# Jackxiini/Pytorch-distributed-learning

Measured on AMD Instinct MI355X. Metric: images/sec (whole node) MNIST ConvNet at 1/2/4/8 MI355X; DDP scaling efficiency, higher is better.
Workload: dtype bf16

## Files before the change

### csrc/kernels/convnet_bwd12.hip

```cpp
#include "convnet_device.h"
#include "convnet_host.h"

namespace ringdp {
namespace kern {

namespace {

__device__ __forceinline__ bf16x8 ones_column_frag(int lane) {
  const bf16 one = (bf16)((lane & 15) == 0 ? 1.f : 0.f);
  return bf16x8{one, one, one, one, one, one, one, one};
}

constexpr int C2_PW = 15, C2_PRS = 80, C2_ORS = 40, C2_DRS = 72;
__constant__ uint8_t c2d_tile_pos[176] = {0,1,2,3,8,9,10,11,12,19,20,13,4,5,6,7,14,15,16,17,22,23,24,25,32,39,34,27,18,33,26,21,28,29,30,31,36,37,38,45,52,53,48,41,46,47,40,35,42,43,44,59,50,51,58,65,66,67,62,55,60,61,54,49,56,57,72,73,64,71,78,79,80,81,76,69,74,75,68,63,70,85,86,87,84,91,92,93,94,95,90,83,88,89,82,77,98,99,100,101,104,105,106,107,108,109,110,111,102,103,96,97,112,113,114,115,118,119,120,121,122,137,130,125,116,123,124,117,126,127,128,129,132,133,134,135,150,151,144,139,136,143,138,131,140,141,142,149,146,147,148,163,164,165,158,153,156,157,152,145,154,155,162,168,160,161,255,255,255,255,255,167,255,255,166,159};
constexpr int C2D_P = C2_PW * C2_PW * C2_PRS * 2;
constexpr int C2D_O = 169 * C2_ORS * 2;
__device__ __forceinline__ int c2_drow(int r) { return (r >> 3) * 704 + (r & 7) * 80; }
constexpr int C2W_D = 16 * 704 * 2;
constexpr int C2W_X = 169 * C2_XRS * 2;
constexpr int C2B_LDS = (C2D_P + 2 * C2D_O) > (C2W_D + C2W_X) ? (C2D_P + 2 * C2D_O) : (C2W_D + C2W_X);
constexpr int C2_WSLAB = 288 * 64 + 64;

__device__ __forceinline__ void conv2_dgrad_role(char* smem, const bf16* __restrict__ dz2, const bf16* __restrict__ packed,
                                 bf16* __restrict__ da1, int B, int block, int nblocks) {
  bf16* P = reinterpret_cast<bf16*>(smem);
  bf16* O = reinterpret_cast<bf16*>(smem + C2D_P);
  const int tid = threadIdx.x, lane = tid & 63, wave = tid >> 6;
  const int nt = wave & 1, mg = wave >> 1;
  const int r16 = lane & 15, q8 = (lane >> 4) * 8;
  const bf16x8* pk = reinterpret_cast<const bf16x8*>(packed + P2D_OFF);
  bf16x8 bw[18];
#pragma unroll
  for (int ks = 0; ks < 18; ++ks) bw[ks] = pk[(nt * 18 + ks) * 64 + lane];
  int base[3];
  int opos[3][4];
#pragma unroll
  for (int k = 0; k < 3; ++k) {
    const int mt = min(mg + 4 * k, 10);
    const int mm = c2d_tile_pos[mt * 16 + r16] == 255 ? 0 : c2d_tile_pos[mt * 16 + r16];
    base[k] = (mm / 13) * C2_PW + mm % 13;
#pragma unroll
    for (int i = 0; i < 4; ++i) opos[k][i] = c2d_tile_pos[mt * 16 + (lane >> 4) * 4 + i];
  }
  for (int c = tid; c < C2D_P / 16; c += 512) reinterpret_cast<bf16x8*>(P)[c] = zero_bf16x8();
  auto copy_out = [&](int bb, const bf16* src) {
    bf16x8* dst = reinterpret_cast<bf16x8*>(da1 + (int64_t)bb * 169 * 32);
    for (int c = tid; c < 676; c += 512) dst[c] = *reinterpret_cast<const bf16x8*>(src + (c >> 2) * C2_ORS + (c & 3) * 8);
  };
  bf16x8 pz[2];
  auto load = [&](int bb) {
    const bf16x8* src = reinterpret_cast<const bf16x8*>(dz2 + (int64_t)bb * 121 * 64);
    pz[0] = src[tid];
    if (tid + 512 < 968) pz[1] = src[tid + 512];
  };
  auto mfma_phase = [&](auto nk_c, bf16* Oc) {
    constexpr int NK = decltype(nk_c)::value;
    f32x4 acc[NK];
#pragma unroll
    for (int k = 0; k < NK; ++k) acc[k] = zero_f32x4();
#pragma unroll
    for (int ks = 0; ks < 18; ++ks) {
      const int tapp = ks >> 1, c0 = (ks & 1) * 32;
      const int shift = (tapp / 3) * C2_PW + tapp % 3;
#pragma unroll
      for (int k = 0; k < NK; ++k)
        acc[k] = mfma16x16x32(*reinterpret_cast<const bf16x8*>(P + (base[k] + shift) * C2_PRS + c0 + q8), bw[ks],
                              acc[k]);
    }
#pragma unroll
    for (int k = 0; k < NK; ++k) {
#pragma unroll
      for (int i = 0; i < 4; ++i) {
        const int m = opos[k][i];
        if (m < 169) Oc[m * C2_ORS + nt * 16 + r16] = (bf16)acc[k][i];
      }
    }
  };
  int b = block, prev = -1, cur = 0;
  if (b < B) load(b);
  for (; b < B; b += nblocks) {
    __syncthreads();
    if (prev >= 0) copy_out(prev, O + (cur ^ 1) * 169 * C2_ORS);
#pragma unroll
    for (int k = 0; k < 2; ++k) {
      const int c = tid + 512 * k;
      if (c < 968) {
        const int pos = c >> 3, cc = (c & 7) * 8;
        *reinterpret_cast<bf16x8*>(P + ((pos / 11 + 2) * C2_PW + pos % 11 + 2) * C2_PRS + cc) = pz[k];
      }
    }
    const int nb = b + nblocks;
    if (nb < B) load(nb);
    __syncthreads();
// ... 350 lines not shown
      if (mg < 3) phase(I3{}, T{}, k);
      else phase(I2{}, T{}, k);
    }
  }
  __syncthreads();
  if (b != block) {
#pragma unroll
    for (int j = 0; j < 4; ++j) c1_step(j, k ^ 1);
  }
  __syncthreads();
  float* red = reinterpret_cast<float*>(smem);
#pragma unroll
  for (int m = 0; m < 2; ++m)
#pragma unroll
    for (int n = 0; n < 2; ++n)
      *reinterpret_cast<f32x4*>(red + ((wave * 4 + m * 2 + n) * 64 + lane) * 4) = acc1[m][n];
  __syncthreads();
  if (tid >= 256) return;
  const int tile = tid >> 6;
  f32x4 sum = *reinterpret_cast<const f32x4*>(red + (tile * 64 + lane) * 4);
#pragma unroll
  for (int w = 1; w < 8; ++w) sum += *reinterpret_cast<const f32x4*>(red + ((w * 4 + tile) * 64 + lane) * 4);
  float* slab = slabs1 + (int64_t)block * C1_WSLAB;
  const int tap = (tile & 1) * 16 + i16;
#pragma unroll
  for (int r = 0; r < 4; ++r) {
    const int co = (tile >> 1) * 16 + g * 4 + r;
    if (tap < 25) slab[co * 25 + tap] = sum[r];
    if (tap == 25) slab[800 + co] = sum[r];
  }
}

template <bool U8>
__global__ __launch_bounds__(512) void conv12_bwd_kernel(const void* __restrict__ xin,
                                                         const uint8_t* __restrict__ idx1,
                                                         const bf16* __restrict__ a1,
                                                         const bf16* __restrict__ dz2,
                                                         const bf16* __restrict__ packed, int B,
                                                         float mean, float inv_std, float in_scale,
                                                         float* __restrict__ slabs2, int nslices,
                                                         float* __restrict__ slabs1, int n_dgrad) {
  __shared__ __attribute__((aligned(16))) char smem[C12B_LDS];
  if ((int)blockIdx.x < n_dgrad)
    conv12_dgrad_role<U8>(smem, xin, idx1, dz2, packed, B, blockIdx.x, n_dgrad, mean, inv_std, in_scale, slabs1);
  else
    conv2_wgrad_role(smem, a1, dz2, slabs2, B, nslices, blockIdx.x - n_dgrad);
}

constexpr int C12V_DG = 2 * (C2D_P + C12_O) + 3 * (C12_XS + C1I_IMG);
constexpr int C12V_WG = 3 * (C2W_D + C2W_X);
constexpr int C12V_LDS = C12V_DG > C12V_WG ? C12V_DG : C12V_WG;
static_assert(C12V_LDS <= 160 * 1024 && C1I_IMG % 16 == 0, "conv12 backward (8-wave) LDS");

#ifndef RINGDP_C12_ABLATE
#define RINGDP_C12_ABLATE 0
#endif
constexpr int C12_ABLATE = RINGDP_C12_ABLATE;

#ifdef RINGDP_C12_STAMPS
constexpr int C12_ST_S0 = 100, C12_ST_BLK = 5, C12_ST_BYTES = 8 * 8 * 4 * 8;
#define C12_ST(s, k) CN_STAMP(C12V_LDS, C12_ST_S0, 4, s, k)
#else
constexpr int C12_ST_BYTES = 0;
#define C12_ST(s, k) do {} while (0)
#endif

template <bool U8>
__device__ __forceinline__ void conv12_dgrad8_role(char* smem, const void* __restrict__ xin,
                                                   const uint8_t* __restrict__ idx1, const bf16* __restrict__ dz2,
                                                   const bf16* __restrict__ packed, int B, int block, int nblocks,
                                                   float mean, float inv_std, float in_scale,
                                                   float* __restrict__ slabs1, int ablate) {
  auto Pb = [&](int k) { return reinterpret_cast<bf16*>(smem + k * C2D_P); };
  auto Ob = [&](int k) { return reinterpret_cast<bf16*>(smem + 2 * C2D_P + k * C12_O); };
  auto Xb = [&](int k) { return reinterpret_cast<bf16*>(smem + 2 * (C2D_P + C12_O) + k * C12_XS); };
  auto Cb = [&](int k) { return reinterpret_cast<uint8_t*>(smem + 2 * (C2D_P + C12_O) + 3 * C12_XS + k * C1I_IMG); };
  const int tid = threadIdx.x, lane = tid & 63;
  const int wave = __builtin_amdgcn_readfirstlane(tid >> 6);
  const int n = block < B ? (B - block + nblocks - 1) / nblocks : 0;
  for (int c = tid; c < (2 * (C2D_P + C12_O) + 3 * C12_XS) / 16; c += 512)
    reinterpret_cast<bf16x8*>(smem)[c] = zero_bf16x8();
  __syncthreads();
  if ((ablate & 8) && wave >= 4) __builtin_amdgcn_s_setprio(1);
  constexpr int C12_KM = 2, C12_KM3 = 4, C12_KH = 26 - 3 * C12_KM - C12_KM3;
  static_assert(C12_KH >= 4 && C12_KM >= 0 && C12_KM3 >= 0, "conv1 k-step partition");
  const int k0 = wave < 4 ? C12_KH + wave * C12_KM : wave - 4, kst = wave < 4 ? 1 : 4;
  const int kcnt = wave < 3 ? C12_KM : wave == 3 ? C12_KM3 : (C12_KH - (wave - 4) + 3) / 4;
  const int i16 = lane & 15, g = lane >> 4, q = i16 >> 2, p = i16 & 3;
  const int t1 = 16 + i16;
  const int xoff0 = (i16 % 5) * C1W_CS + (i16 / 5) * C1W_RS + 8 * g;
  const int xoff1 = t1 < 25 ? (t1 % 5) * C1W_CS + (t1 / 5) * C1W_RS + 8 * g : 0;
  const uint32_t b1fill = t1 == 25 ? 0x3f803f80u : 0u;
  f32x4 acc1[2][2];
#pragma unroll
  for (int m = 0; m < 2; ++m) acc1[m][0] = acc1[m][1] = zero_f32x4();
  const int o_lane = ((4 * g + q) * C2_ORS + 4 * p) * 2;
  const int c_lane = (i16 >> 1) * 16 + 4 * g, csh_lane = 4 * (i16 & 1);
  struct C1F {
    uint2 d[2];
    uint32_t cu[2];
    bf16x8 b0, b1;
  };
  auto c1_read = [&](int ks, int oimg, int ximg, int cimg, C1F& f) {
    const int py = ks >> 1;
    int oa = oimg + py * (13 * C2_ORS * 2) + o_lane, ca = cimg + py * 256 + c_lane;
    int x0 = ximg + ks * (C1W_RS * 2) + xoff0 * 2, x1 = ximg + ks * (C1W_RS * 2) + xoff1 * 2;
    asm("" : "+v"(oa), "+v"(ca), "+v"(x0), "+v"(x1));
#pragma unroll
    for (int m = 0; m < 2; ++m) {
      f.d[m] = __builtin_bit_cast(uint2, lds_read_tr16(reinterpret_cast<const bf16*>(smem + oa) + m * 16));
      f.cu[m] = *reinterpret_cast<const uint32_t*>(smem + ca + m * 128);
    }
    f.b0 = *reinterpret_cast<const bf16x8*>(smem + x0);
    f.b1 = *reinterpret_cast<const bf16x8*>(smem + x1);
  };
  auto c1_mma = [&](int ks, const C1F& f) {
    bf16x8 A[2];
    const int csh = csh_lane + 2 * (ks & 1);
#pragma unroll
    for (int m = 0; m < 2; ++m) {
      const uint2 d = f.d[m];
      const uint32_t cu = f.cu[m];
      uint32_t pr[4];
#pragma unroll
      for (int e = 0; e < 4; ++e) {
        const uint32_t dv = e & 1 ? (e < 2 ? d.x : d.y) >> 16 : (e < 2 ? d.x : d.y) & 0xffffu;
        const uint32_t sel = __builtin_amdgcn_ubfe(cu, 8 * e + csh, 2);
        pr[e] = dv * ((sel * 0x8001u) & 0x10001u);
      }
      A[m] = __builtin_bit_cast(bf16x8, make_uint4(pr[0], pr[1], pr[2], pr[3]));
    }
    bf16x8 B1 = f.b1;
    if (t1 >= 25) B1 = __builtin_bit_cast(bf16x8, make_uint4(b1fill, b1fill, b1fill, b1fill));
#pragma unroll
    for (int m = 0; m < 2; ++m) {
      acc1[m][0] = mfma16x16x32(A[m], f.b0, acc1[m][0]);
      acc1[m][1] = mfma16x16x32(A[m], B1, acc1[m][1]);
    }
  };
  auto c1_image = [&](int j) {
    const int oimg = 2 * C2D_P + (j & 1) * C12_O;
    const int ximg = 2 * (C2D_P + C12_O) + (j % 3) * C12_XS;
    const int cimg = 2 * (C2D_P + C12_O) + 3 * C12_XS + (j % 3) * C1I_IMG;
    for (int i = 0, ks = k0; i < kcnt; ++i, ks += kst) {
      C1F f;
      c1_read(ks, oimg, ximg, cimg, f);
      c1_mma(ks, f);
    }
  };
  if (wave < 4) {
    const int r16 = lane & 15, q8 = (lane >> 4) * 8, c4 = (lane >> 4) * 4;
    const bf16x8* pk = reinterpret_cast<const bf16x8*>(packed + P2D_OFF);
    bf16x8 bw[2][18];
#pragma unroll
    for (int nt = 0; nt < 2; ++nt)
#pragma unroll
      for (int ks = 0; ks < 18; ++ks) bw[nt][ks] = pk[(nt * 18 + ks) * 64 + lane];
    int base[3], opos[3];
#pragma unroll
    for (int k = 0; k < 3; ++k) {
      const int mt = min(wave + 4 * k, 10);
      const int mm = c2d_tile_pos[mt * 16 + r16];
      opos[k] = mm;
      base[k] = mm == 255 ? 0 : (mm / 13) * C2_PW + mm % 13;
    }
    auto phase = [&](auto nk_c, const bf16* P, bf16* O, int s) {
      constexpr int NK = decltype(nk_c)::value;
      f32x4 acc[NK][2];
#pragma unroll
      for (int k = 0; k < NK; ++k) acc[k][0] = acc[k][1] = zero_f32x4();
#pragma unroll
      for (int ks = 0; ks < 18; ++ks) {
        const int tapp = ks >> 1, c0 = (ks & 1) * 32;
        const int shift = (tapp / 3) * C2_PW + tapp % 3;
#pragma unroll
        for (int k = 0; k < NK; ++k) {
          const bf16x8 a = *reinterpret_cast<const bf16x8*>(P + (base[k] + shift) * C2_PRS + c0 + q8);
          acc[k][0] = mfma16x16x32(bw[0][ks], a, acc[k][0]);
          acc[k][1] = mfma16x16x32(bw[1][ks], a, acc[k][1]);
        }
      }
      C12_ST(s, 1);
#pragma unroll
      for (int k = 0; k < NK; ++k) {
        if (opos[k] < 169) {
#pragma unroll
          for (int nt = 0; nt < 2; ++nt)
            *reinterpret_cast<bf16x4*>(O + opos[k] * C2_ORS + nt * 16 + c4) =
                bf16x4{(bf16)acc[k][nt][0], (bf16)acc[k][nt][1], (bf16)acc[k][nt][2], (bf16)acc[k][nt][3]};
        }
      }
    };
    lds_barrier();
    for (int s = 0; s <= n; ++s) {
      C12_ST(s, 0);
      if (s < n && !(ablate & 2)) {
        if (wave < 3)
          phase(std::integral_constant<int, 3>{}, Pb(s & 1), Ob(s & 1), s);
        else
          phase(std::integral_constant<int, 2>{}, Pb(s & 1), Ob(s & 1), s);
      }
      C12_ST(s, 2);
      if (s >= 1 && !(ablate & 1)) c1_image(s - 1);
      C12_ST(s, 3);
      lds_barrier();
    }
  } else {
    const int vt = tid - 256;
    struct Regs {
      bf16x8 pz[4];
      uint4 pc;
      uint32_t xu;
      float4 xf;
    };
    Regs r0, r1;
    auto load = [&](Regs& r, int bb) {
      const bf16x8* src = reinterpret_cast<const bf16x8*>(dz2 + (int64_t)bb * 121 * 64);
#pragma unroll
      for (int j = 0; j < 4; ++j)
        if (vt + 256 * j < 968) r.pz[j] = src[vt + 256 * j];
      if (vt < C1I_IMG / 16) r.pc = reinterpret_cast<const uint4*>(idx1 + (int64_t)bb * C1I_IMG)[vt];
      c1_load<U8>(xin, bb, vt, r.xu, r.xf);
    };
    auto stage = [&](const Regs& r, int k2, int k3) {
      bf16* P = Pb(k2);
#pragma unroll
      for (int j = 0; j < 4; ++j) {
        const int c = vt + 256 * j;
        if (c < 968) {
          const int pos = c >> 3, cc = (c & 7) * 8;
// ... 163 lines not shown
      C12_ST(i, 1);
      if (!early && i + 2 < n) {
        stage(rs, (i + 2) % 3);
        if (i + 4 < n) load(rs, img(i + 4));
      }
      lds_barrier();
      C12_ST(i, 2);
    };
    for (int i = 0; i < n; i += 2) {
      image(i, r0);
      if (i + 1 < n) image(i + 1, r1);
    }
  };
  if (h == 0)
    body(std::integral_constant<int, 0>{});
  else
    body(std::integral_constant<int, 1>{});
  float* slab = slabs + (int64_t)slice * C2_WSLAB;
  const int nj = h == 0 ? 5 : 4;
#pragma unroll
  for (int m = 0; m < 2; ++m) {
    const int co = (2 * wm2 + m) * 16 + grp * 4;
#pragma unroll
    for (int j = 0; j < 5; ++j) {
      if (j < nj) {
        const int nn = ((2 * j + h) * 2 + half) * 16 + g16;
        *reinterpret_cast<f32x4*>(slab + (int64_t)nn * 64 + co) = acc[m][j];
      }
    }
    if (wn == 0 && g16 == 0) *reinterpret_cast<f32x4*>(slab + 288 * 64 + co) = accb[m];
  }
}

template <bool U8>
__global__ __launch_bounds__(512, 1) void conv12_bwd8_kernel(const void* __restrict__ xin,
                                                            const uint8_t* __restrict__ idx1,
                                                            const bf16* __restrict__ a1,
                                                            const bf16* __restrict__ dz2,
                                                            const bf16* __restrict__ packed, int B, float mean,
                                                            float inv_std, float in_scale,
                                                            float* __restrict__ slabs2, int nslices,
                                                            float* __restrict__ slabs1, int n_dgrad, int ablate) {
  __shared__ __attribute__((aligned(16))) char smem[C12V_LDS + C12_ST_BYTES];
  if ((int)blockIdx.x < n_dgrad)
    conv12_dgrad8_role<U8>(smem, xin, idx1, dz2, packed, B, blockIdx.x, n_dgrad, mean, inv_std, in_scale, slabs1,
                           ablate);
  else if (!(ablate & 4))
    conv2_wgrad8_role(smem, a1, dz2, slabs2, B, nslices, blockIdx.x - n_dgrad);
#ifdef RINGDP_C12_STAMPS
  __syncthreads();
  const bool dg = (int)blockIdx.x < n_dgrad;
  const int blk = dg ? blockIdx.x : blockIdx.x - n_dgrad, nb = dg ? n_dgrad : nslices;
  if (blk == C12_ST_BLK && threadIdx.x == 0 && (B - blk) / nb > C12_ST_S0 + 8) {
    const unsigned long long* st = reinterpret_cast<const unsigned long long*>(smem + C12V_LDS);
    const unsigned long long t0 = st[0];
    for (int w = 0; w < 8; ++w)
      for (int k = 0; k < 8; ++k) {
        const unsigned long long* r = st + (w * 8 + k) * 4;
        printf("C12ST %c w%d s%d %lld %lld %lld %lld\n", dg ? 'd' : 'w', w, k, (long long)(r[0] - t0),
               (long long)(r[1] - t0), (long long)(r[2] - t0), dg ? (long long)(r[3] - t0) : 0ll);
      }
  }
#endif
}

}

static void c2_split(int B, bool dgrad, int& nd, int& ws) {
  const int cus = num_cus();
  if (!dgrad) {
    nd = 0;
    ws = clampi(cdiv(B, 8), 1, cus);
    return;
  }
  static const double frac = env_real("RINGDP_C2_DGRAD_FRAC", 0.55, split_frac_ok);
  nd = clampi(B, 1, (int)(frac * cus));
  const int per = cdiv(B, nd);
  ws = clampi(cdiv(B, std::max(per, 2)), 1, std::max(1, cus - nd));
}

static void c12_split(int B, int& nd, int& ws) {
  const int cus = num_cus();
  if (use_8wave(B)) {
    static const double frac3 = env_real("RINGDP_C12_DGRAD_FRAC", 0.59, split_frac_ok);
    nd = clampi(((int)(frac3 * cus) + 4) / 8 * 8, 8, cus - 8);
    ws = clampi(cdiv(B, 8), 1, cus - nd);
    return;
  }
  static const double frac = env_real("RINGDP_C12_DGRAD_FRAC", 0.64, split_frac_ok);
  static const int wmin = env_int("RINGDP_C12_WMIN", 2, slab_images_ok);
  nd = clampi(B, 1, (int)(frac * cus));
  const int per = cdiv(B, nd);
  ws = clampi(cdiv(B, std::max(per, wmin)), 1, std::max(1, cus - nd));
}

static int conv1_wslices(int B) { return clampi(cdiv(B, 4), 1, 3 * num_cus()); }

int64_t cn_conv2_slab_floats(int B, bool dgrad) {
  int nd, ws;
  c2_split(B, dgrad, nd, ws);
  return (int64_t)ws * C2_WSLAB;
}
int64_t cn_conv12_slab_floats(int B) {
  int nd, ws;
  c12_split(B, nd, ws);
  return (int64_t)ws * C2_WSLAB + (int64_t)nd * C1_WSLAB;
}
int64_t cn_conv1_slab_floats(int B) { return (int64_t)conv1_wslices(B) * C1_WSLAB; }

void cn_conv2_bwd(const void* a1, const void* dz2, const void* packed, void* da1, int B, float* slabs,
                  float* dw2, float* db2, hipStream_t s) {
  int nd, ws;
  c2_split(B, da1 != nullptr, nd, ws);
  conv2_bwd_kernel<<<nd + ws, 512, 0, s>>>(static_cast<const bf16*>(a1), static_cast<const bf16*>(dz2),
                                           static_cast<const bf16*>(packed), static_cast<bf16*>(da1), B, slabs,
                                           ws, nd);
  launch_reduce({seg(slabs, C2_WSLAB, 0, 288 * 64, ws, dw2, 1, 32, 64), seg(slabs, C2_WSLAB, 288 * 64, 64, ws, db2)},
                s);
}

void cn_conv12_bwd(const void* x, bool u8, const uint8_t* idx1, const void* a1, const void* dz2,
                   const void* packed, int B, float mean, float inv_std, float in_scale, float* slabs, float* dw2,
                   float* db2, float* dw1, float* db1, hipStream_t s, const ReduceList* extra) {
  int nd, ws;
  c12_split(B, nd, ws);
  float *slabs2 = slabs, *slabs1 = slabs + (int64_t)ws * C2_WSLAB;
  const bf16 *a1b = static_cast<const bf16*>(a1), *dzb = static_cast<const bf16*>(dz2),
             *pk = static_cast<const bf16*>(packed);
  dispatch_bool(u8, [&](auto U8) {
    if (use_8wave(B))
      conv12_bwd8_kernel<decltype(U8)::value><<<nd + ws, 512, 0, s>>>(x, idx1, a1b, dzb, pk, B, mean, inv_std, in_scale,
                                                                      slabs2, ws, slabs1, nd, C12_ABLATE);
    else
      conv12_bwd_kernel<decltype(U8)::value><<<nd + ws, 512, 0, s>>>(x, idx1, a1b, dzb, pk, B, mean, inv_std, in_scale,
                                                                     slabs2, ws, slabs1, nd);
  });
  ReduceList r = extra ? *extra : ReduceList{};
  for (const ReduceSeg& g : {seg(slabs2, C2_WSLAB, 0, 288 * 64, ws, dw2, 1, 32, 64),
                             seg(slabs2, C2_WSLAB, 288 * 64, 64, ws, db2), seg(slabs1, C1_WSLAB, 0, 800, nd, dw1),
                             seg(slabs1, C1_WSLAB, 800, 32, nd, db1)})
    r.push_back(g);
  launch_reduce(r, s);
}

void cn_conv1_wgrad(const void* x, bool u8, const void* da1, const uint8_t* idx1, int B, float mean,
                    float inv_std, float in_scale, float* slabs, float* dw1, float* db1, hipStream_t s) {
  const int ws = conv1_wslices(B);
  dispatch_bool(u8, [&](auto U8) {
    conv1_wgrad_kernel<decltype(U8)::value><<<ws, 256, 0, s>>>(x, static_cast<const bf16*>(da1), idx1, B, mean, inv_std,
                                                               in_scale, slabs, ws);
  });
  launch_reduce({seg(slabs, C1_WSLAB, 0, 800, ws, dw1), seg(slabs, C1_WSLAB, 800, 32, ws, db1)}, s);
}

}
}
```

### csrc/kernels/convnet_bwd3.hip

```cpp
#include "convnet_device.h"
#include "convnet_host.h"

namespace ringdp::kern {
namespace {
__host__ __device__ inline int fc_imgs(int B) { return B <= 1024 ? 4 : (B >= 65536 ? 128 : (B >= 32768 ? 64 : 32)); }
constexpr int FC_SLAB = 10 * 2048 + 10 + 128 + 2;

template <bool kCE>
__device__ __forceinline__ void fc_bwd_body(const bf16* __restrict__ a3, const bf16* __restrict__ packed,
                                            const float* __restrict__ dl, bf16* __restrict__ da3m,
                                            float* __restrict__ slabs, int B, int imgs, const CeFuse& ce, int blk) {
  const int t = threadIdx.x;
  const int wd = t >> 4, co0 = (t & 15) * 8;
  float wr[8][10];
  {
    const bf16x8* src = reinterpret_cast<const bf16x8*>(packed + PFC_OFF + (wd * 128 + co0) * 10);
#pragma unroll
    for (int h = 0; h < 10; ++h) {
      const bf16x8 v = src[h];
#pragma unroll
      for (int e = 0; e < 8; ++e) wr[(8 * h + e) / 10][(8 * h + e) % 10] = (float)v[e];
    }
  }
  float acc[8][10];
// ... 361 lines not shown
                                                           const uint8_t* __restrict__ idx3,
                                                           const bf16* __restrict__ packed, bf16* __restrict__ dz2,
                                                           int B, float* __restrict__ slabs, int n_wgrad,
                                                           int n_dgrad, int b_dgrad, int n_fc,
                                                           float* __restrict__ fc_slabs, int fc_n_imgs) {
  __shared__ __attribute__((aligned(16))) char smem[C3B_LDS];
  int blk = blockIdx.x;
  if (blk < n_fc) {
    if (src.dl)
      fc_bwd_body<false>(src.a3, packed, src.dl, nullptr, fc_slabs, B, fc_n_imgs, src.ce, blk);
    else
      fc_bwd_body<true>(src.a3, packed, nullptr, nullptr, fc_slabs, B, fc_n_imgs, src.ce, blk);
    return;
  }
  blk -= n_fc;
  int b_first = blk, b_end = b_dgrad, b_step = n_dgrad;
  if (blk >= n_dgrad) {
    const int w = blk - n_dgrad;
    conv3_wgrad_role(smem, a2, src, idx3, slabs, B, n_wgrad, w >> 1, w & 1);
    if (dz2 == nullptr || b_dgrad >= B) return;
    __syncthreads();
    b_first = b_dgrad + w;
    b_end = B;
    b_step = 2 * n_wgrad;
  }
  conv3_dgrad_role(smem, src, idx3, idx2, packed, dz2, b_first, b_end, b_step);
}

constexpr int C3S_B = 2048 * 2 + 2048;
constexpr int C3V_DA = 100 * 64 * 4;
constexpr int C3V_FV = 8 * 64 * 16;
constexpr int C3V_F = C3V_FV + 8 * 64 * 4;
constexpr int C3V_XRS = 80;
constexpr int C3V_X = 100 * C3V_XRS * 2;
constexpr int C3V_DG = 2 * (C3D_P + C3V_DA + C3D_AM + C3S_B);
constexpr int C3V_WG = 3 * C3V_X + 2 * C3V_F + 2 * C3S_B;
constexpr int C3V_LDS = C3V_DG > C3V_WG ? C3V_DG : C3V_WG;
static_assert(C3V_LDS <= 160 * 1024 && C3V_F % 16 == 0 && C3V_X % 16 == 0, "conv3 backward (8-wave) LDS");
__device__ __forceinline__ int c3v_da(int p, int x, int k) { return p * 64 + ((k ^ (2 * (x & 7))) << 2); }
template <int J>
__device__ __forceinline__ float ubyte_f32(uint32_t v) {
  float r;
  if constexpr (J == 0) asm("v_cvt_f32_ubyte0 %0, %1" : "=v"(r) : "v"(v));
  else if constexpr (J == 1) asm("v_cvt_f32_ubyte1 %0, %1" : "=v"(r) : "v"(v));
  else if constexpr (J == 2) asm("v_cvt_f32_ubyte2 %0, %1" : "=v"(r) : "v"(v));
  else asm("v_cvt_f32_ubyte3 %0, %1" : "=v"(r) : "v"(v));
  return r;
}

template <int N>
__device__ __forceinline__ float dpp_row_shr(float v) {
  return __int_as_float(__builtin_amdgcn_update_dpp(0, __float_as_int(v), 0x110 + N, 0xf, 0xf, true));
}

__device__ __forceinline__ void c3s_glds(const bf16* __restrict__ da3m, const uint8_t* __restrict__ idx3, int b,
                                         char* S, int k, int lane) {
  const uint32_t voff = ((k & 3) * 64 + lane) * 16;
  if (k < 4)
    glds16_sv(da3m + (int64_t)b * 2048, voff, S + k * 1024);
  else
    glds16_sv(idx3 + (int64_t)b * 2048, voff, S + k * 1024);
}

__device__ __forceinline__ void c3s_pre(const char* S, int tid, C3Pre& p) {
  if (tid < 256) {
    p.da = reinterpret_cast<const bf16x8*>(S)[tid];
    p.id = reinterpret_cast<const uint2*>(S + 4096)[tid];
  }
}

__device__ __forceinline__ uint32_t c3w_stage_off(int k, int lane) {
  if (k < 4) return (k * 64 + (lane & ~15) + ((lane & 15) ^ (2 * k))) * 16;
  const int kk = k - 4;
  return (kk * 64 + (lane & ~7) + ((lane & 7) ^ (2 * kk + (lane >> 5)))) * 16;
}
__device__ __forceinline__ void c3w_stage_glds(const bf16* __restrict__ da3m, const uint8_t* __restrict__ idx3, int b,
                                               char* S, int k, uint32_t voff) {
  if (k < 4)
    glds16_sv(da3m + (int64_t)b * 2048, voff, S + k * 1024);
  else
    glds16_sv(idx3 + (int64_t)b * 2048, voff, S + k * 1024);
}

typedef __bf16 bf16x16 __attribute__((ext_vector_type(16)));
__device__ __forceinline__ f32x4 smfmac16x16x64(const bf16x8& a, const bf16x16& b, const f32x4& c, int idx) {
  return __builtin_amdgcn_smfmac_f32_16x16x64_bf16(a, b, c, idx, 0, 0);
}

__device__ __forceinline__ uint32_t a2_rows_off(int k, int lane) {
  const int c = k * 64 + lane;
  if (c >= 1000) return ~0u;
  const int row = c / 10, sub = c - 10 * row;
  return (row * 64 + (sub & 7) * 8) * 2;
}
__device__ __forceinline__ void a2_glds_rows(const bf16* __restrict__ a2, int b, bf16* X, int k, uint32_t voff) {
  if (voff != ~0u) glds16_sv(a2 + (int64_t)b * 6400, voff, X + k * 512);
}

struct C3Pool2Map {
  int dst;
  int daA[9], daB[9];
  int amA[9], amB[9];
  int sh[8][4];
  bool eight;
};
__device__ __forceinline__ void c3_pool2_map(int hwave, int lane, C3Pool2Map& m) {
  const int q = (lane >> 2) & 7;
  const int run = 4 * hwave + 2 * (lane >> 5) + (__builtin_popcount(q) & 1), k = (q >> 1) * 4 + (lane & 3);
  const int p0 = run < 9 ? 8 * run : 7 * run + 9;
  m.eight = run < 9;
  m.dst = p0 * 64 + k * 4;
  int gy = p0 / 11, x = p0 - 11 * gy;
  auto entry = [&](int e, int xc) {
    const int rowA = min(gy, 9), rowB = max(gy - 1, 0);
    m.daA[e] = c3v_da(rowA * 10 + xc, xc, k);
    m.daB[e] = c3v_da(rowB * 10 + xc, xc, k);
    m.amA[e] = rowA * 640 + xc * 64 + k * 4;
    m.amB[e] = rowB * 640 + xc * 64 + k * 4;
  };
  entry(0, max(x - 1, 0));
#pragma unroll
  for (int i = 0; i < 8; ++i) {
    entry(i + 1, min(x, 9));
    const int sA = gy <= 9 ? 0 : 4, sB = gy >= 1 ? 2 : 4;
    m.sh[i][0] = x < 10 ? sA : 4;
    m.sh[i][1] = x > 0 ? sA + 1 : 4;
    m.sh[i][2] = x < 10 ? sB : 4;
    m.sh[i][3] = x > 0 ? sB + 1 : 4;
    if (++x == 11) {
      x = 0;
      ++gy;
    }
  }
}
__device__ __forceinline__ void c3_pool2_bwd(const C3Pool2Map& m, const float* DA, const uint8_t* AM,
                                             bf16* __restrict__ dz2_img) {
  auto masked_add = [](f32x4& g, uint32_t cw, int sh, const f32x4& d) {
    const uint32_t mk = (cw >> sh) & 0x01010101u;
    g[0] = fmaf(d[0], ubyte_f32<0>(mk), g[0]);
    g[1] = fmaf(d[1], ubyte_f32<1>(mk), g[1]);
    g[2] = fmaf(d[2], ubyte_f32<2>(mk), g[2]);
    g[3] = fmaf(d[3], ubyte_f32<3>(mk), g[3]);
  };
  auto code = [&](int off) { return *reinterpret_cast<const uint32_t*>(AM + off); };
  auto da2 = [&](int off) { return *reinterpret_cast<const f32x4*>(DA + off); };
  bf16x4* dst = reinterpret_cast<bf16x4*>(dz2_img + m.dst);
  uint32_t pa = code(m.amA[0]), pb = code(m.amB[0]);
  f32x4 qa = da2(m.daA[0]), qb = da2(m.daB[0]);
#pragma unroll
  for (int i = 0; i < 8; ++i) {
    if (i == 7 && !m.eight) break;
    const uint32_t na = code(m.amA[i + 1]), nb2 = code(m.amB[i + 1]);
    const f32x4 ea = da2(m.daA[i + 1]), eb = da2(m.daB[i + 1]);
    f32x4 g = zero_f32x4();
    masked_add(g, na, m.sh[i][0], ea);
    masked_add(g, pa, m.sh[i][1], qa);
    masked_add(g, nb2, m.sh[i][2], eb);
    masked_add(g, pb, m.sh[i][3], qb);
    dst[i * 16] = bf16x4{(bf16)g[0], (bf16)g[1], (bf16)g[2], (bf16)g[3]};
    pa = na;
    pb = nb2;
    qa = ea;
    qb = eb;
  }
}
constexpr int C3_POOL2_DMA_WAVE_STORES = 7;

#ifndef RINGDP_C3_ABLATE
#define RINGDP_C3_ABLATE 0
#endif
constexpr int C3_ABLATE = RINGDP_C3_ABLATE;
// ... 366 lines not shown
```

### csrc/kernels/convnet_device.h

```cpp
#pragma once

#include "device_common.h"

namespace ringdp::kern {
using namespace ringdp::dev;
namespace {

constexpr int P1_OFF = 0, P1_N = 2 * 2 * 512;
constexpr int P2F_OFF = P1_OFF + P1_N, P2F_N = 4 * 9 * 512;
constexpr int P3F_OFF = P2F_OFF + P2F_N, P3F_N = 8 * 18 * 512;
constexpr int P2D_OFF = P3F_OFF + P3F_N, P2D_N = 2 * 18 * 512;
constexpr int P3D_OFF = P2D_OFF + P2D_N, P3D_N = 4 * 36 * 512;
constexpr int PFC_OFF = P3D_OFF + P3D_N, PFC_N = 16 * 128 * 10;
constexpr int PFF_OFF = PFC_OFF + PFC_N, PFF_N = 64 * 64 * 8;
constexpr int PACK_TOTAL = PFF_OFF + PFF_N;

__device__ __forceinline__ int win_pos(int r, int pw) {
  const int w = r >> 2, i = r & 3;
  return (2 * (w >> 2) + (i >> 1)) * pw + 2 * (w & 3) + (i & 1);
}

__device__ __forceinline__ void glds16_async(const void* gsrc, void* lds_wave_base) {
  const unsigned base = __builtin_amdgcn_readfirstlane(
      (unsigned)(size_t)((__attribute__((address_space(3))) char*)(lds_wave_base)));
  asm volatile("s_mov_b32 m0, %0\n\ts_nop 0\n\tglobal_load_lds_dwordx4 %1, off" ::"s"(base), "v"(gsrc) : "memory");
}
__device__ __forceinline__ void c_dma_wait() { asm volatile("s_waitcnt vmcnt(0)" ::: "memory"); }
template <int N>
__device__ __forceinline__ void c_dma_wait_but() { asm volatile("s_waitcnt vmcnt(%0)" ::"n"(N) : "memory"); }

__device__ __forceinline__ void glds16_sv(const void* sbase, uint32_t voff, void* lds_wave_base) {
  const unsigned base = __builtin_amdgcn_readfirstlane(
      (unsigned)(size_t)((__attribute__((address_space(3))) char*)(lds_wave_base)));
  asm volatile("s_mov_b32 m0, %0\n\ts_nop 0\n\tglobal_load_lds_dwordx4 %1, %2" ::"s"(base), "v"(voff), "s"(sbase)
               : "memory");
}

__device__ __forceinline__ void lds_barrier() { asm volatile("s_waitcnt lgkmcnt(0)\n\ts_barrier" ::: "memory"); }

constexpr int C3_XRS = 72;

__device__ __forceinline__ void a2_glds(const bf16* __restrict__ a2, int b, bf16* R, int wave, int lane,
                                        int nwaves) {
  const bf16* src = a2 + (int64_t)b * 6400;
  for (int k = wave; k < 13; k += nwaves) {
    const int slot = k * 64 + lane;
    if (slot < 800) glds16_async(src + slot * 8, R + k * 512);
  }
}

template <int RS = C3_XRS>
__device__ __forceinline__ void a2_relayout(const bf16* R, bf16* X, int tid, int nthreads) {
  for (int c = tid; c < 800; c += nthreads)
    *reinterpret_cast<bf16x8*>(X + (c >> 3) * RS + (c & 7) * 8) = reinterpret_cast<const bf16x8*>(R)[c];
}

constexpr int XC_W = 32, XC_SZ = 30 * XC_W;

template <bool U8>
__device__ __forceinline__ void c1_load(const void* xin, int b, int tid, uint32_t& u, float4& f) {
  if (tid < 196) {
    if (U8)
      u = reinterpret_cast<const uint32_t*>(static_cast<const uint8_t*>(xin) + (int64_t)b * 784)[tid];
    else
      f = reinterpret_cast<const float4*>(static_cast<const float*>(xin) + (int64_t)b * 784)[tid];
  }
}

template <bool U8, int NC, int RS = XC_W, int CS = XC_SZ>
__device__ __forceinline__ void c1_store(bf16* xc, int tid, uint32_t u, float4 f, float mean, float inv_std,
                                         float in_scale) {
  if (tid < 196) {
    float v[4];
    if (U8) {
#pragma unroll
      for (int k = 0; k < 4; ++k) v[k] = (float)((u >> (8 * k)) & 0xff) * in_scale;
    } else {
      v[0] = f.x;
      v[1] = f.y;
      v[2] = f.z;
      v[3] = f.w;
    }
    bf16 xv[4];
#pragma unroll
    for (int k = 0; k < 4; ++k) xv[k] = (bf16)((v[k] - mean) * inv_std);
    const uint32_t lo16 = __builtin_bit_cast(uint16_t, xv[0]), m1 = __builtin_bit_cast(uint16_t, xv[1]),
                   m2 = __builtin_bit_cast(uint16_t, xv[2]), hi16 = __builtin_bit_cast(uint16_t, xv[3]);
    const uint32_t p01 = lo16 | (m1 << 16), p23 = m2 | (hi16 << 16), p12 = m1 | (m2 << 16);
    const int pr = tid / 7 + 1, pc0 = 4 * (tid % 7) + 1;
#pragma unroll
    for (int s = 0; s < NC; ++s) {
      bf16* d = xc + s * CS + pr * RS + pc0 - s;
      if ((s & 3) == 1) {
        *reinterpret_cast<uint2*>(d) = make_uint2(p01, p23);
      } else if ((s & 3) == 3) {
        reinterpret_cast<uint32_t*>(d)[0] = p01;
        reinterpret_cast<uint32_t*>(d)[1] = p23;
      } else {
        d[0] = xv[0];
        *reinterpret_cast<uint32_t*>(d + 1) = p12;
        d[3] = xv[3];
      }
    }
  }
}

constexpr int C1I_IMG = 13 * 256;
constexpr int C1A_IMG = 169 * 32;
constexpr int C2_XRS = 48;

#define CN_STAMP(lds_end, s0, slots, s, k)                                                                         \
  do {                                                                                                             \
    if ((s) >= (s0) && (s) < (s0) + 8 && (threadIdx.x & 63) == 0)                                                  \
      reinterpret_cast<unsigned long long*>(smem + (lds_end))[((threadIdx.x >> 6) * 8 + ((s) - (s0))) * (slots) + (k)] = \
          __builtin_amdgcn_s_memtime();                                                                            \
  } while (0)

}
}
```

Measured before the change: 20.91 million.

## Use sparse SMFMAC 16x16x64 for conv1 weight-gradient through maxpool mask

The conv1 weight-gradient inner loop now exploits the 2:4 sparsity of the maxpool-routed gradient. It packs only the selected entries and builds sparsity indices from the pool selector bits, then issues smfmac_f32_16x16x64_bf16 in place of dense mfma16x16x32. Each step now covers a pooled row pair, which halves the step count, and the k-step partition across waves is rebalanced accordingly. The dgrad/wgrad CU split fraction is lowered from 0.59 to 0.56 to match the cheaper conv1 work. This risks correctness if the index encoding is wrong, and it raises register use for the doubled fragments.

```diff
diff --git a/csrc/kernels/convnet_bwd12.hip b/csrc/kernels/convnet_bwd12.hip
--- a/csrc/kernels/convnet_bwd12.hip
+++ b/csrc/kernels/convnet_bwd12.hip
@@ -9,6 +9,11 @@
 __device__ __forceinline__ bf16x8 ones_column_frag(int lane) {
   const bf16 one = (bf16)((lane & 15) == 0 ? 1.f : 0.f);
   return bf16x8{one, one, one, one, one, one, one, one};
+}
+
+typedef unsigned short u16x2 __attribute__((ext_vector_type(2)));
+__device__ __forceinline__ uint32_t pk_mul_u16(uint32_t a, uint32_t b) {
+  return __builtin_bit_cast(uint32_t, __builtin_bit_cast(u16x2, a) * __builtin_bit_cast(u16x2, b));
 }
 
 constexpr int C2_PW = 15, C2_PRS = 80, C2_ORS = 40, C2_DRS = 72;
@@ -525,10 +530,10 @@
     reinterpret_cast<bf16x8*>(smem)[c] = zero_bf16x8();
   __syncthreads();
   if ((ablate & 8) && wave >= 4) __builtin_amdgcn_s_setprio(1);
-  constexpr int C12_KM = 2, C12_KM3 = 4, C12_KH = 26 - 3 * C12_KM - C12_KM3;
-  static_assert(C12_KH >= 4 && C12_KM >= 0 && C12_KM3 >= 0, "conv1 k-step partition");
-  const int k0 = wave < 4 ? C12_KH + wave * C12_KM : wave - 4, kst = wave < 4 ? 1 : 4;
-  const int kcnt = wave < 3 ? C12_KM : wave == 3 ? C12_KM3 : (C12_KH - (wave - 4) + 3) / 4;
+  constexpr int C12_S3 = 1, C12_SH = 13 - C12_S3;
+  static_assert(C12_SH >= 4 && C12_S3 >= 0, "conv1 step partition");
+  const int k0 = wave < 4 ? C12_SH : wave - 4, kst = wave < 4 ? 1 : 4;
+  const int kcnt = wave < 3 ? 0 : wave == 3 ? C12_S3 : (C12_SH - (wave - 4) + 3) / 4;
   const int i16 = lane & 15, g = lane >> 4, q = i16 >> 2, p = i16 & 3;
   const int t1 = 16 + i16;
   const int xoff0 = (i16 % 5) * C1W_CS + (i16 / 5) * C1W_RS + 8 * g;
@@ -537,58 +542,68 @@
   f32x4 acc1[2][2];
 #pragma unroll
   for (int m = 0; m < 2; ++m) acc1[m][0] = acc1[m][1] = zero_f32x4();
-  const int o_lane = ((4 * g + q) * C2_ORS + 4 * p) * 2;
-  const int c_lane = (i16 >> 1) * 16 + 4 * g, csh_lane = 4 * (i16 & 1);
+  const int o_lane = ((8 * (g & 1) + q) * C2_ORS + 4 * p) * 2;
+  const int c_lane = (i16 >> 1) * 16 + 8 * (g & 1);
+  const uint32_t csh = 4 * (i16 & 1) + 2 * (g >> 1);
   struct C1F {
-    uint2 d[2];
-    uint32_t cu[2];
-    bf16x8 b0, b1;
-  };
-  auto c1_read = [&](int ks, int oimg, int ximg, int cimg, C1F& f) {
-    const int py = ks >> 1;
+    uint2 d[2][2];
+    uint2 cu[2];
+    bf16x8 b0[2], b1[2];
+  };
+  auto c1_read = [&](int py, int oimg, int ximg, int cimg, C1F& f) {
     int oa = oimg + py * (13 * C2_ORS * 2) + o_lane, ca = cimg + py * 256 + c_lane;
-    int x0 = ximg + ks * (C1W_RS * 2) + xoff0 * 2, x1 = ximg + ks * (C1W_RS * 2) + xoff1 * 2;
+    int x0 = ximg + py * (2 * C1W_RS * 2) + xoff0 * 2, x1 = ximg + py * (2 * C1W_RS * 2) + xoff1 * 2;
     asm("" : "+v"(oa), "+v"(ca), "+v"(x0), "+v"(x1));
 #pragma unroll
     for (int m = 0; m < 2; ++m) {
-      f.d[m] = __builtin_bit_cast(uint2, lds_read_tr16(reinterpret_cast<const bf16*>(smem + oa) + m * 16));
-      f.cu[m] = *reinterpret_cast<const uint32_t*>(smem + ca + m * 128);
-    }
-    f.b0 = *reinterpret_cast<const bf16x8*>(smem + x0);
-    f.b1 = *reinterpret_cast<const bf16x8*>(smem + x1);
-  };
-  auto c1_mma = [&](int ks, const C1F& f) {
+#pragma unroll
+      for (int h = 0; h < 2; ++h)
+        f.d[m][h] = __builtin_bit_cast(
+            uint2, lds_read_tr16(reinterpret_cast<const bf16*>(smem + oa) + h * 4 * C2_ORS + m * 16));
+      f.cu[m] = *reinterpret_cast<const uint2*>(smem + ca + m * 128);
+    }
+#pragma unroll
+    for (int h = 0; h < 2; ++h) {
+      f.b0[h] = *reinterpret_cast<const bf16x8*>(smem + x0 + h * C1W_RS * 2);
+      f.b1[h] = *reinterpret_cast<const bf16x8*>(smem + x1 + h * C1W_RS * 2);
+    }
+  };
+  auto c1_mma = [&](const C1F& f) {
     bf16x8 A[2];
-    const int csh = csh_lane + 2 * (ks & 1);
+    int ix[2];
 #pragma unroll
     for (int m = 0; m < 2; ++m) {
-      const uint2 d = f.d[m];
-      const uint32_t cu = f.cu[m];
-      uint32_t pr[4];
-#pragma unroll
-      for (int e = 0; e < 4; ++e) {
-        const uint32_t dv = e & 1 ? (e < 2 ? d.x : d.y) >> 16 : (e < 2 ? d.x : d.y) & 0xffffu;
-        const uint32_t sel = __builtin_amdgcn_ubfe(cu, 8 * e + csh, 2);
-        pr[e] = dv * ((sel * 0x8001u) & 0x10001u);
-      }
-      A[m] = __builtin_bit_cast(bf16x8, make_uint4(pr[0], pr[1], pr[2], pr[3]));
-    }
-    bf16x8 B1 = f.b1;
-    if (t1 >= 25) B1 = __builtin_bit_cast(bf16x8, make_uint4(b1fill, b1fill, b1fill, b1fill));
+      const uint32_t ux = f.cu[m].x >> csh, uy = f.cu[m].y >> csh;
+      const uint32_t lx = (ux | (ux >> 1)) & 0x01010101u, ly = (uy | (uy >> 1)) & 0x01010101u;
+      A[m] = __builtin_bit_cast(
+          bf16x8, make_uint4(pk_mul_u16(f.d[m][0].x, __builtin_amdgcn_perm(0u, lx, 0x0c010c00u)),
+                             pk_mul_u16(f.d[m][0].y, __builtin_amdgcn_perm(0u, lx, 0x0c030c02u)),
+                             pk_mul_u16(f.d[m][1].x, __builtin_amdgcn_perm(0u, ly, 0x0c010c00u)),
+                             pk_mul_u16(f.d[m][1].y, __builtin_amdgcn_perm(0u, ly, 0x0c030c02u))));
+      const uint32_t E = ((ux >> 1) & 0x01010101u) | (uy & 0x02020202u);
+      const uint32_t G = ((__umul24(E, 0x1041u) >> 12) & 0x3fu) | ((E >> 18) & 0xc0u);
+      ix[m] = (int)((G & 0x55u) | ((G & 0xaau) << 7) | 0x8888u);
+    }
+    bf16x16 B0 = __builtin_shufflevector(f.b0[0], f.b0[1], 0, 1, 2, 3, 4, 5, 6, 7, 8, 9, 10, 11, 12, 13, 14, 15);
+    bf16x16 B1 = __builtin_shufflevector(f.b1[0], f.b1[1], 0, 1, 2, 3, 4, 5, 6, 7, 8, 9, 10, 11, 12, 13, 14, 15);
+    if (t1 >= 25) {
+      const bf16x8 fill = __builtin_bit_cast(bf16x8, make_uint4(b1fill, b1fill, b1fill, b1fill));
+      B1 = __builtin_shufflevector(fill, fill, 0, 1, 2, 3, 4, 5, 6, 7, 8, 9, 10, 11, 12, 13, 14, 15);
+    }
 #pragma unroll
     for (int m = 0; m < 2; ++m) {
-      acc1[m][0] = mfma16x16x32(A[m], f.b0, acc1[m][0]);
-      acc1[m][1] = mfma16x16x32(A[m], B1, acc1[m][1]);
+      acc1[m][0] = smfmac16x16x64(A[m], B0, acc1[m][0], ix[m]);
+      acc1[m][1] = smfmac16x16x64(A[m], B1, acc1[m][1], ix[m]);
     }
   };
   auto c1_image = [&](int j) {
     const int oimg = 2 * C2D_P + (j & 1) * C12_O;
     const int ximg = 2 * (C2D_P + C12_O) + (j % 3) * C12_XS;
     const int cimg = 2 * (C2D_P + C12_O) + 3 * C12_XS + (j % 3) * C1I_IMG;
-    for (int i = 0, ks = k0; i < kcnt; ++i, ks += kst) {
+    for (int i = 0, py = k0; i < kcnt; ++i, py += kst) {
       C1F f;
-      c1_read(ks, oimg, ximg, cimg, f);
-      c1_mma(ks, f);
+      c1_read(py, oimg, ximg, cimg, f);
+      c1_mma(f);
     }
   };
   if (wave < 4) {
@@ -918,7 +933,7 @@
 static void c12_split(int B, int& nd, int& ws) {
   const int cus = num_cus();
   if (use_8wave(B)) {
-    static const double frac3 = env_real("RINGDP_C12_DGRAD_FRAC", 0.59, split_frac_ok);
+    static const double frac3 = env_real("RINGDP_C12_DGRAD_FRAC", 0.56, split_frac_ok);
     nd = clampi(((int)(frac3 * cus) + 4) / 8 * 8, 8, cus - 8);
     ws = clampi(cdiv(B, 8), 1, cus - nd);
     return;
diff --git a/csrc/kernels/convnet_bwd3.hip b/csrc/kernels/convnet_bwd3.hip
--- a/csrc/kernels/convnet_bwd3.hip
+++ b/csrc/kernels/convnet_bwd3.hip
@@ -467,11 +467,6 @@
     glds16_sv(idx3 + (int64_t)b * 2048, voff, S + k * 1024);
 }
 
-typedef __bf16 bf16x16 __attribute__((ext_vector_type(16)));
-__device__ __forceinline__ f32x4 smfmac16x16x64(const bf16x8& a, const bf16x16& b, const f32x4& c, int idx) {
-  return __builtin_amdgcn_smfmac_f32_16x16x64_bf16(a, b, c, idx, 0, 0);
-}
-
 __device__ __forceinline__ uint32_t a2_rows_off(int k, int lane) {
   const int c = k * 64 + lane;
   if (c >= 1000) return ~0u;
diff --git a/csrc/kernels/convnet_device.h b/csrc/kernels/convnet_device.h
--- a/csrc/kernels/convnet_device.h
+++ b/csrc/kernels/convnet_device.h
@@ -37,6 +37,11 @@
 }
 
 __device__ __forceinline__ void lds_barrier() { asm volatile("s_waitcnt lgkmcnt(0)\n\ts_barrier" ::: "memory"); }
+
+typedef __bf16 bf16x16 __attribute__((ext_vector_type(16)));
+__device__ __forceinline__ f32x4 smfmac16x16x64(const bf16x8& a, const bf16x16& b, const f32x4& c, int idx) {
+  return __builtin_amdgcn_smfmac_f32_16x16x64_bf16(a, b, c, idx, 0, 0);
+}
 
 constexpr int C3_XRS = 72;
 
```

After: 21.26 million, median of 6. +1.7%, better.
